# eivindeb/fixed-wing-gym

Hardware: AMD Instinct MI355X
Metric: env-steps/sec (higher is better)
Workload: dtype f32

## Files before the change

fixed-wing-gym_amd/csrc/fwgym.hip:

```cpp
#include <math.h>
#include <stdio.h>
#include <string.h>
#include <string>
#include <vector>
#include "fwgym_env.h"
#include "fwgym_actor.h"
#include "fwgym_learner.h"
#include "fwgym_eval.h"

__device__ __forceinline__ float wave_sum(float v) { return wave_sum64(v); }

struct SpecWords { unsigned w[sizeof(DevCfg) / 4]; };
static_assert(sizeof(SpecWords) == sizeof(DevCfg), "DevCfg must be made of 32-bit members only");
#if defined(FWG_SPECS_FILE)
#include FWG_SPECS_FILE
#elif defined(FWG_WITH_SPECS)
#include "generated/specs.inc"
#else
#define FWG_SPEC_LIST(X)
#endif
#ifndef FWG_SHAPE_LIST
#define FWG_SHAPE_LIST(X)
#endif
#define FWG_SHAPE_BASE FWG_INSTANCE_SHAPE
// ... 1053 lines not shown
    return rollout_shared_floats(c, hsplit) + actor_scratch_floats() + FWG_RO_ENVS * 4;
}
template <bool TURB, int SPEC, int HSPLIT>
__global__ __launch_bounds__(2 * FWG_RO_ENVS, 2) void k_rollout(const DevCfg* __restrict__ cp, const DynCfg* __restrict__ dp, const KArgs A0,
                                                                 const ActorArgs AA) {
    extern __shared__ __attribute__((aligned(16))) float lds[];
    const DevCfg& c = SpecCfg<SPEC>::get(cp);
    constexpr int NK1 = (SpecCfg<SPEC>::obs_dim + 15) / 16;
    const int shared = rollout_shared_floats(c, HSPLIT);
    ActorLds Z;
    Z.F = reinterpret_cast<frag_t*>(lds);
    Z.mean_s = lds + shared;
    Z.rstd_s = Z.mean_s + FWG_ACT_MAX_OBS;
    Z.misc = Z.rstd_s + FWG_ACT_MAX_OBS;
    Z.bias = Z.misc + 4 + 2 * FWG_ACT_MAX_OBS + 4;
    Z.act_out = lds + shared + actor_scratch_floats();
    const unsigned act_ctr = actor_block<HSPLIT, NK1>(AA, Z, (long)blockIdx.x * FWG_RO_ENVS);
    FWG_BLOCK_SYNC_LDS();
    const int wave = threadIdx.x >> 6, group = wave & (FWG_RO_GROUPS - 1);
    const int sub = (int)blockIdx.x * FWG_RO_GROUPS + group;
    const HeadStats hs{Z.mean_s, Z.misc[1], act_ctr + 1u};
    float* area = lds + group * lds_map(c.obs_dim, c.n_obs, c.L.window, c.use_cmd_ring, false, c.obs_log, true).total;
    const float* acts = Z.act_out + group * (FWG_WAVE * 4);
    if (wave < FWG_RO_GROUPS) step_wave<TURB, SPEC, 1, HeadStats>(cp, dp, A0, area, sub, acts, hs);
    else step_wave<TURB, SPEC, 2, HeadStats>(cp, dp, A0, area, sub, acts, hs);
}

template <bool TURB, int SPEC>
__global__ __launch_bounds__(FWG_WAVE) void k_reset(const DevCfg* __restrict__ cp, const DynCfg* __restrict__ dp, const KArgs A0) {
    extern __shared__ __attribute__((aligned(16))) float lds[];
// ... 894 lines not shown
    return FWG_OK;
}

int fwg_reduce_success_device(fwg_handle* h, float* out_dev, void* stream) {
    if (!h || !out_dev) return fail_with(FWG_ERR_INVALID, "null argument");
    launch_finish(h, h->last_metrics_out, (hipStream_t)stream);
    hipLaunchKernelGGL(k_reduce_take, dim3(1), dim3(FWG_WAVE), 0, (hipStream_t)stream, h->d_reduce, out_dev);
    HIP_TRY(hipGetLastError());
    return FWG_OK;
}

int fwg_spec_index(const fwg_handle* h) { return h ? h->spec : -1; }
#ifdef FWG_TIMELINE
int fwg_debug_set_trace(fwg_handle* h, long long* trace_dev) { if (!h) return FWG_ERR_INVALID; h->trace = trace_dev; return FWG_OK; }
int fwg_debug_set_actor_trace(struct fwg_actor* a, long long* trace_dev);
#endif

int fwg_set_graph_mode(fwg_handle* h, int enable, void* stream) {
    if (!h) return fail_with(FWG_ERR_INVALID, "null handle");
    HIP_TRY(hipStreamSynchronize((hipStream_t)stream));
    if (enable) {
        StepSlots s[2];
        s[h->gstep & 1] = host_slots(h, h->gstep);
        s[(h->gstep + 1) & 1] = host_slots(h, h->gstep - 1);
        HIP_TRY(hipMemcpy(h->d_slots, s, sizeof(s), hipMemcpyHostToDevice));
    } else if (h->graph_mode) {
        StepSlots s[2];
        HIP_TRY(hipMemcpy(s, h->d_slots, sizeof(s), hipMemcpyDeviceToHost));
        h->gstep = s[0].gnow > s[1].gnow ? s[0].gnow : s[1].gnow;
    }
// ... 89 lines not shown
static void launch(const fwg_handle* h, const KArgs& A, hipStream_t stream) {
    if (with_instance(h->spec, [&](auto inst) { launch_one<IS_STEP, decltype(inst)::TURB, decltype(inst)::SPEC>(h, A, stream); })) return;
#ifndef FWG_DEV_FAST_BUILD
    if (h->h.turbulence) launch_one<IS_STEP, true, -1>(h, A, stream);
    else launch_one<IS_STEP, false, -1>(h, A, stream);
#endif
}


struct fwg_actor {
    int device;
    int64_t n_envs, env_base;
    int D, act_dim, nk1;
    float gamma, clip_obs, clip_rew, eps;
    int training, precise, parity;
    uint64_t seed;
    ActorStats* d_stats;
    unsigned long long* d_acc;
    int acc_cols;
    frag_t* d_frags;
    float* d_bias;
    float* d_log_std;
    float* d_ret;
    size_t lds_act[2];
    int cnn_filters, cnn_rows;
    size_t lds_cnn[2];
    const fwg_handle* log_env;
#ifdef FWG_TIMELINE
    long long* trace;
#endif
// ... 26 lines not shown

static ActorArgs act_args(const fwg_actor* a, const float* obs, const float* reward, const uint8_t* done, float* norm_obs_out, float* action_out,
                          float* value_out, float* logp_out, float* norm_reward_out, uint8_t* done_out, int deterministic) {
    ActorArgs A = actor_args(a);
    A.obs = obs; A.rew = reward; A.done = done;
    A.norm_obs = norm_obs_out; A.action = action_out; A.value = value_out; A.logp = logp_out; A.norm_rew = norm_reward_out;
    A.done_out = done_out; A.deterministic = deterministic ? 1 : 0;
    return A;
}
typedef void (*actor_kernel_t)(ActorArgs);
static actor_kernel_t actor_kernel(int precise, int nk1) {
    static const actor_kernel_t table[2][4] = {{k_actor_act<1, 1>, k_actor_act<1, 2>, k_actor_act<1, 3>, k_actor_act<1, 4>},
                                               {k_actor_act<3, 1>, k_actor_act<3, 2>, k_actor_act<3, 3>, k_actor_act<3, 4>}};
    return table[precise ? 1 : 0][nk1 - 1];
}

static bool rollout_fits(const fwg_handle* h);
static bool rollout_grant_lds(const fwg_handle* h);

static void observer_args(const fwg_handle* h, KArgs* A) {
    const fwg_actor* a = h->observer;
    if (!a) return;
    A->acc = a->d_acc;
    A->acc_ctr = &a->d_stats[a->parity].act_counter;
    A->acc_mean = a->d_stats[a->parity].mean; A->acc_ret_mean = &a->d_stats[a->parity].ret_mean;
    A->acc_ret = a->d_ret; A->acc_gamma = a->gamma; A->acc_cols = a->acc_cols;
}

extern "C" {

int fwg_attach_observer(fwg_handle* h, fwg_actor* a) {
    if (!h) return fail_with(FWG_ERR_INVALID, "fwg_attach_observer: null env handle");
    if (a && h->h.obs_log > 0)
        return fail_with(FWG_ERR_INVALID, "fwg_attach_observer: row-log observations keep the lagged rows out of the step kernel; use fwg_actor_observe");
    if (a && (a->n_envs != h->n_envs || a->D != h->h.obs_dim || a->device != h->device))
        return fail_with(FWG_ERR_INVALID, "fwg_attach_observer: the head was created for another batch size / observation size / device");
    h->observer = a;
    h->rollout_lds_granted = 0;
    if (a && h->spec >= 0 && h->split && rollout_fits(h)) h->rollout_lds_granted = rollout_grant_lds(h) ? 1 : 0;
    return FWG_OK;
}

#ifdef FWG_TIMELINE
int fwg_debug_set_actor_trace(fwg_actor* a, long long* trace_dev) { if (!a) return FWG_ERR_INVALID; a->trace = trace_dev; return FWG_OK; }
#endif
int fwg_actor_set_obs_log(fwg_actor* a, const fwg_handle* env) {
    if (!a) return fail_with(FWG_ERR_INVALID, "fwg_actor_set_obs_log: null actor");
    if (env != nullptr) {
        if (env->h.obs_log <= 0) return fail_with(FWG_ERR_INVALID, "fwg_actor_set_obs_log: the env writes the dense observation batch");
        if (env->n_envs != a->n_envs || env->h.obs_dim != a->D || env->device != a->device || (env->h.n_obs & 3))
            return fail_with(FWG_ERR_INVALID, "fwg_actor_set_obs_log: batch size / observation size / device mismatch (n_obs must be a multiple of 4)");
        if (a->cnn_filters && env->h.n_obs * a->cnn_rows != a->D)
            return fail_with(FWG_ERR_INVALID, "fwg_actor_set_obs_log: the CNN head's conv spans a window of another length than the env's");
    }
    a->log_env = env;
    return FWG_OK;
}

int fwg_actor_create(int device, int64_t n_envs, int obs_dim, int act_dim, float gamma, float clip_obs, float clip_reward,
                     float epsilon, fwg_actor** out) {
    if (!out) return fail_with(FWG_ERR_INVALID, "fwg_actor_create: null argument");
    if (n_envs < 1) return fail_with(FWG_ERR_INVALID, "fwg_actor_create: n_envs < 1");
    if (obs_dim < 1 || obs_dim > FWG_ACT_MAX_OBS) return fail_with(FWG_ERR_INVALID, "fwg_actor_create: obs_dim must be in [1, 64]");
    if (act_dim < 1 || act_dim > FWG_ACT_MAX_ACT) return fail_with(FWG_ERR_INVALID, "fwg_actor_create: act_dim must be in [1, 4]");
    HIP_TRY(hipSetDevice(device));
    fwg_actor* a = new fwg_actor();
    memset(a, 0, sizeof(*a));
    a->device = device; a->n_envs = n_envs; a->D = obs_dim; a->act_dim = act_dim; a->nk1 = (obs_dim + 15) / 16;
    a->gamma = gamma; a->clip_obs = clip_obs; a->clip_rew = clip_reward; a->eps = epsilon;
    a->training = 1; a->precise = 1;
    a->acc_cols = acc_cols_for(obs_dim);
    a->lds_act[0] = actor_lds_bytes(a->nk1, 1);
    a->lds_act[1] = actor_lds_bytes(a->nk1, 2);
    const int rc = [&]() -> int {
        const size_t nfrag = (size_t)2 * 2 * actor_frags(a->nk1) * 64;
        HIP_TRY(hipMalloc((void**)&a->d_stats, 2 * sizeof(ActorStats)));
        const size_t acc_bytes = (size_t)FWG_ACC_SETS * FWG_ACC_SHARDS * a->acc_cols * sizeof(unsigned long long);
        HIP_TRY(hipMalloc((void**)&a->d_acc, acc_bytes));
        HIP_TRY(hipMemset(a->d_acc, 0, acc_bytes));
        HIP_TRY(hipMalloc((void**)&a->d_frags, nfrag * sizeof(frag_t)));
        HIP_TRY(hipMalloc((void**)&a->d_bias, (2 * FWG_ACT_BIAS_FLOATS + FWG_CNN_PARAMS) * sizeof(float)));
        HIP_TRY(hipMemset(a->d_bias, 0, (2 * FWG_ACT_BIAS_FLOATS + FWG_CNN_PARAMS) * sizeof(float)));
        HIP_TRY(hipMalloc((void**)&a->d_log_std, FWG_ACT_MAX_ACT * sizeof(float)));
        HIP_TRY(hipMalloc((void**)&a->d_ret, (size_t)n_envs * sizeof(float)));
        HIP_TRY(hipMemset(a->d_frags, 0, nfrag * sizeof(frag_t)));
        HIP_TRY(hipMemset(a->d_log_std, 0, FWG_ACT_MAX_ACT * sizeof(float)));
        HIP_TRY(hipMemset(a->d_ret, 0, (size_t)n_envs * sizeof(float)));
        ActorStats s[2];
        memset(s, 0, sizeof(s));
        for (int p = 0; p < 2; ++p) {
            for (int f = 0; f < FWG_ACT_MAX_OBS; ++f) s[p].var[f] = 1.f;
            s[p].count = 1e-4f; s[p].ret_var = 1.f; s[p].ret_count = 1e-4f;
        }
        HIP_TRY(hipMemcpy(a->d_stats, s, sizeof(s), hipMemcpyHostToDevice));
        for (int precise = 0; precise < 2; ++precise)
            HIP_TRY(hipFuncSetAttribute((const void*)actor_kernel(precise, a->nk1), hipFuncAttributeMaxDynamicSharedMemorySize, (int)a->lds_act[precise]));
        return FWG_OK;
    }();
    if (rc != FWG_OK) { fwg_actor_destroy(a); return rc; }
    *out = a;
    return FWG_OK;
}

void fwg_actor_destroy(fwg_actor* a) {
    if (!a) return;
    (void)hipFree(a->d_stats); (void)hipFree(a->d_acc); (void)hipFree(a->d_frags); (void)hipFree(a->d_bias); (void)hipFree(a->d_log_std); (void)hipFree(a->d_ret);
    delete a;
}

int fwg_actor_set_weights(fwg_actor* a, const fwg_actor_weights* w) {
    if (!a || !w) return fail_with(FWG_ERR_INVALID, "fwg_actor_set_weights: null argument");
// ... 108 lines not shown
    HIP_TRY(hipGetLastError());
    return FWG_OK;
}

int fwg_actor_act(fwg_actor* a, const float* obs, const float* reward, const uint8_t* done, float* norm_obs_out,
                  float* action_out, float* value_out, float* logp_out, float* norm_reward_out, uint8_t* done_out,
                  int deterministic, void* stream) {
    if (!a || !obs) return fail_with(FWG_ERR_INVALID, "fwg_actor_act: null argument");
    HIP_TRY(hipSetDevice(a->device));
    const ActorArgs A = act_args(a, obs, reward, done, norm_obs_out, action_out, value_out, logp_out, norm_reward_out, done_out, deterministic);
    const dim3 grid((unsigned)((a->n_envs + FWG_ACT_ENVS - 1) / FWG_ACT_ENVS)), block(64 * FWG_ACT_WAVES);
    hipStream_t st = (hipStream_t)stream;
    if (a->cnn_filters) {
        if (a->precise) hipLaunchKernelGGL((k_actor_act_cnn<3>), grid, block, a->lds_cnn[1], st, A);
        else hipLaunchKernelGGL((k_actor_act_cnn<1>), grid, block, a->lds_cnn[0], st, A);
    } else hipLaunchKernelGGL(actor_kernel(a->precise, a->nk1), grid, block, a->lds_act[a->precise], st, A);
    HIP_TRY(hipGetLastError());
    a->parity ^= 1;
    return FWG_OK;
}

}
static size_t rollout_lds_bytes(const fwg_handle* h, int hsplit) { return (size_t)rollout_lds_floats(h->h, hsplit) * sizeof(float); }
static bool rollout_fits(const fwg_handle* h) {
    bool ok = false;
    with_instance(h->spec, [&](auto inst) { ok = SpecCfg<decltype(inst)::SPEC>::rollout_ok && rollout_lds_bytes(h, 3) <= 160 * 1024; });
    return ok;
}
static bool rollout_grant_lds(const fwg_handle* h) {
    bool ok = false;
    with_instance(h->spec, [&](auto inst) {
// ... 180 lines not shown
```

fixed-wing-gym_amd/csrc/fwgym_actor.h:

```cpp
#pragma once
#include "fwgym_env.h"

#define FWG_STREAM_POLICY 6u
#define FWG_ACT_BLOCK 256
#define FWG_ACT_WAVES 8
#define FWG_ACT_ENVS (32 * FWG_ACT_WAVES)
#define FWG_ACT_PRESCALE 2.885390081777927f
#define FWG_ACT_MAX_OBS 64
#define FWG_ACT_MAX_ACT 4

struct ActorStats { float mean[FWG_ACT_MAX_OBS], var[FWG_ACT_MAX_OBS]; float count, ret_mean, ret_var, ret_count; unsigned act_counter, pad_[3]; };

struct alignas(16) frag_t { unsigned x, y, z, w; };

struct ActorArgs {
    const float* obs; const float* rew; const uint8_t* done;
    const StepSlots* obs_slots; long long obs_win; int obs_n;
#ifdef FWG_TIMELINE
    long long* trace;
#endif
    float* ret;
    ActorStats* stats;
    unsigned long long* acc; int acc_cols;
    const frag_t* frags;
// ... 49 lines not shown
    return __uint_as_float(u);
#else
    float f; memcpy(&f, &u, 4); return f;
#endif
}

__device__ __forceinline__ const float* actor_obs_at(const ActorArgs& A, long long win, long e, int f0) {
    if (A.obs_n == 0) return A.obs + e * A.D + f0;
    const int r = f0 / A.obs_n, j = f0 - r * A.obs_n;
    return A.obs + ((win + r) * A.N + e) * A.obs_n + j;
}
__device__ __forceinline__ long long actor_obs_win(const ActorArgs& A) { return A.obs_slots != nullptr ? A.obs_slots->log_win : A.obs_win; }

#ifdef FWG_TIMELINE
#define FWG_ATL(A, i) do { if ((A).trace != nullptr) { const long long t_ = __builtin_amdgcn_s_memtime(); asm volatile("" ::: "memory"); \
        if ((threadIdx.x & 63) == 0) (A).trace[(blockIdx.x * FWG_ACT_WAVES + (threadIdx.x >> 6)) * 16 + (i)] = t_; } } while (0)
#else
#define FWG_ATL(A, i) do { } while (0)
#endif

typedef float f32x16 __attribute__((ext_vector_type(16)));
#ifdef FWG_EMU
#define fwg_mfma_bf16(a, b, c) emu_mfma_f32_32x32x16_bf16((a), (b), (c))
#define fwg_exp2(x) exp2f(x)
#else
typedef __bf16 fwg_bf16x8 __attribute__((ext_vector_type(8)));
__device__ __forceinline__ f32x16 fwg_mfma_bf16(const frag_t& a, const frag_t& b, f32x16 c) {
    return __builtin_amdgcn_mfma_f32_32x32x16_bf16(__builtin_bit_cast(fwg_bf16x8, a), __builtin_bit_cast(fwg_bf16x8, b), c, 0, 0, 0);
}
#define fwg_exp2(x) __builtin_amdgcn_exp2f(x)
#endif
// ... 53 lines not shown
__device__ __forceinline__ void mma3s(const frag_t& a_hi, const frag_t& a_lo, const frag_t& b_hi, const frag_t& b_lo, f32x16& acc, f32x16& acc_a,
                                      f32x16& acc_b) {
    if (SPLIT > 1) {
        acc_a = fwg_mfma_bf16(a_lo, b_hi, acc_a);
        acc_b = fwg_mfma_bf16(a_hi, b_lo, acc_b);
    }
    acc = fwg_mfma_bf16(a_hi, b_hi, acc);
}
template <int SPLIT, int NF>
__device__ __forceinline__ void load_frags(const frag_t* F, int nfw, int base, int l, frag_t (&hi)[NF], frag_t (&lo)[NF]) {
#pragma unroll
    for (int i = 0; i < NF; ++i) {
        hi[i] = F[(base + i) * 64 + l];
        if (SPLIT > 1) lo[i] = F[(nfw + base + i) * 64 + l];
    }
}
__device__ __forceinline__ f32x16 bias_tile(const float* b, int it, int half) {
    f32x16 a;
#pragma unroll
    for (int q = 0; q < 4; ++q) {
        const float4 v = *reinterpret_cast<const float4*>(b + 32 * it + 8 * q + 4 * half);
        a[4 * q] = v.x; a[4 * q + 1] = v.y; a[4 * q + 2] = v.z; a[4 * q + 3] = v.w;
    }
    return a;
}

__device__ __forceinline__ void hidden_block(const f32x16& a, int kb, frag_t& hi, frag_t& lo) {
    float x[8];
#if defined(FWG_ABL_TANH_ID)
#pragma unroll
// ... 83 lines not shown
    for (int kk = 0; kk < 4; ++kk) {
        mma3s<SPLIT>(w3_hi[kk], w3_lo[kk], bp_hi[kk], bp_lo[kk], o_pi, oa, ob);
        hidden_block(kk < 2 ? v0 : v1, kk & 1, bv_hi[kk], bv_lo[kk]);
        FWG_SCHED_MFMA_VALU(SPLIT > 1 ? 3 : 1, SPLIT > 1 ? 16 : 48);
        FWG_SCHED_FENCE();
    }
    FWG_ATL(A, 12);
    load_frags<SPLIT, 4>(FV, nfw, 2 * NK1 + 8, l, w3_hi, w3_lo);
    o_vf = bias_tile(bV + 128, 0, half);
    f32x16 va = {0.f}, vb = {0.f};
#pragma unroll
    for (int kk = 0; kk < 4; ++kk) mma3s<SPLIT>(w3_hi[kk], w3_lo[kk], bv_hi[kk], bv_lo[kk], o_vf, va, vb);
    if (SPLIT > 1) {
#pragma unroll
        for (int i = 0; i < 4; ++i) { o_pi[i] += oa[i] + ob[i]; o_vf[i] += va[i] + vb[i]; }
    }
}

__global__ __launch_bounds__(FWG_ACT_BLOCK) void k_actor_stats(const ActorArgs A) {
    const int tid = threadIdx.x, lane = tid & 63;
    const long e = (long)blockIdx.x * FWG_ACT_BLOCK + tid;
    const bool valid = e < A.N;
    const long wave = e >> 6;
    if ((wave << 6) >= A.N) return;
    const ActorStats& S = A.stats[A.parity];
    const int D = A.D;
    const bool has_obs = A.obs != nullptr, has_ret = A.rew != nullptr;
    float dr = 0.f;
    if (has_ret && valid) {
        const float r = A.ret[e] * A.gamma + A.rew[e];
// ... 8 lines not shown
        float v[32];
#pragma unroll
        for (int i = 0; i < 32; ++i) v[i] = FWG_ACC_COLUMN(32 * chunk + i, D, valid, FWG_OBS_AT, S.mean, dr, has_obs, has_ret);
        acc_flush(acc, A.acc_cols, (int)(wave & (FWG_ACC_SHARDS - 1)), chunk, lane, wave_totals32(v, lane));
    }
#undef FWG_OBS_AT
}

struct ActorLds {
    frag_t* F;
    float* mean_s;
    float* rstd_s;
    float* misc;
    float* act_out;
    float* bias;
};
__host__ __device__ inline int actor_weight_floats(int nk1, int parts) { return 2 * parts * actor_frags(nk1) * 64 * 4; }
__host__ __device__ inline int actor_scratch_floats() { return 2 * FWG_ACT_MAX_OBS + 4 + 2 * FWG_ACT_MAX_OBS + 4 + 2 * FWG_ACT_BIAS_FLOATS; }

template <int SPLIT, int NK1, bool CNN = false>
__device__ __forceinline__ unsigned actor_block(const ActorArgs& A, const ActorLds& Z, long env_first) {
    const int tid = threadIdx.x, l = tid & 63, wv = tid >> 6, j = l & 31, half = l >> 5;
    constexpr int nf = 2 * NK1 + 12;
    constexpr int PARTS = SPLIT > 1 ? 2 : 1;
    const bool first_block = env_first == 0;
    FWG_ATL(A, 0);
    frag_t* F = Z.F;
    float* mean_s = Z.mean_s;
    float* rstd_s = Z.rstd_s;
    float* misc = Z.misc;
    constexpr int n_pieces = PARTS == 2 ? 2 * 2 * nf : 2 * nf;
    constexpr int per_wave = (n_pieces + FWG_ACT_WAVES - 1) / FWG_ACT_WAVES;
    float4 wreg[per_wave];
#ifndef FWG_ABL_ACT_NO_STAGE
#pragma unroll
    for (int i = 0; i < per_wave; ++i) {
        const int q = wv + i * FWG_ACT_WAVES;
        wreg[i] = make_float4(0.f, 0.f, 0.f, 0.f);
        if (q < n_pieces) {
            const int src = PARTS == 2 ? q : ((q / nf) * 2 * nf + (q % nf));
            wreg[i] = reinterpret_cast<const float4*>(A.frags + src * 64)[l];
        }
    }
#endif
    const long e = env_first + wv * 32 + j;
    const bool valid = e < A.N;
    const bool vec4 = (A.D & 3) == 0 && (A.obs_n & 3) == 0;
    const long long win = actor_obs_win(A);
    constexpr int NRAW = CNN ? FWG_CNN_ROWS * FWG_CNN_COLS / 4 : 1;
    float4 raw_w[NRAW];
    float cnn_p[CNN ? FWG_CNN_PARAMS : 1];
    if constexpr (CNN) {
#pragma unroll
        for (int q = 0; q < NRAW; ++q) raw_w[q] = valid ? *reinterpret_cast<const float4*>(actor_obs_at(A, win, e, 4 * q)) : make_float4(0.f, 0.f, 0.f, 0.f);
#pragma unroll
        for (int i = 0; i < FWG_CNN_PARAMS; ++i) cnn_p[i] = A.bias[2 * FWG_ACT_BIAS_FLOATS + i];
    }
    float raw_x[CNN ? 1 : NK1][8];
#pragma unroll
    for (int kk = 0; kk < (CNN ? 0 : NK1); ++kk) {
// ... 2 lines not shown
            const int f0 = k_input(kk, half, 4 * q);
            float v[4] = {0.f, 0.f, 0.f, 0.f};
            if (valid && f0 < A.D) {
                if (vec4) {
                    const float4 g = *reinterpret_cast<const float4*>(actor_obs_at(A, win, e, f0));
                    v[0] = g.x; v[1] = g.y; v[2] = g.z; v[3] = g.w;
                } else {
#pragma unroll
                    for (int i = 0; i < 4; ++i) if (f0 + i < A.D) v[i] = A.obs[e * A.D + f0 + i];
                }
            }
#pragma unroll
            for (int i = 0; i < 4; ++i) raw_x[kk][4 * q + i] = v[i];
        }
    }
    const unsigned act_ctr = A.stats[A.parity].act_counter;
    const float bias_in = tid < 2 * FWG_ACT_BIAS_FLOATS ? A.bias[tid] : 0.f;
    float ls_in[FWG_ACT_MAX_ACT];
#pragma unroll
    for (int i = 0; i < FWG_ACT_MAX_ACT; ++i) ls_in[i] = i < A.act_dim ? A.log_std[i] : 0.f;
    const float rew_in = (A.rew != nullptr && valid) ? A.rew[e] : 0.f;
    const uint8_t done_in = (A.done != nullptr && valid) ? A.done[e] : (uint8_t)0;
    FWG_ATL(A, 1);
    {
        const ActorStats& S0 = A.stats[A.parity];
        ActorStats& S1 = A.stats[A.parity ^ 1];
        const int D = A.D, cols = 2 * D + 4;
        const size_t set_words = (size_t)FWG_ACC_SHARDS * A.acc_cols;
        const unsigned long long* acc = A.acc + (size_t)(act_ctr % FWG_ACC_SETS) * set_words;
        float* tot = misc + 4;
        if (tid < cols) {
            long long sum = 0;
#pragma unroll
            for (int sh = 0; sh < FWG_ACC_SHARDS; ++sh) sum += (long long)acc[(long)sh * A.acc_cols + tid];
            tot[tid] = (tid == 2 || tid == 3) ? (float)sum : (float)sum * (1.f / FWG_ACC_SCALE);
        }
        if (tid < 2 * FWG_ACT_BIAS_FLOATS) Z.bias[tid] = bias_in;
        FWG_BLOCK_SYNC_LDS();
        const float n_obs = A.training ? tot[2] : 0.f, n_ret = A.training ? tot[3] : 0.f;
        if (tid < FWG_ACT_MAX_OBS) {
            const int f = tid;
            float m = 0.f, rs = 0.f, v = 1.f;
            if (f < D) {
                m = S0.mean[f]; v = S0.var[f];
                if (n_obs > 0.f) {
                    const float cnt = S0.count, tt = cnt + n_obs;
                    const float s1 = tot[4 + 2 * f] / n_obs, s2 = tot[5 + 2 * f] / n_obs;
                    const float bvar = fmaxf(s2 - s1 * s1, 0.f);
                    const float mm = v * cnt + bvar * n_obs + s1 * s1 * (cnt * n_obs / tt);
                    m += s1 * (n_obs / tt);
                    v = mm / tt;
                }
                rs = 1.f / sqrtf(v + A.eps);
            }
            mean_s[f] = m; rstd_s[f] = rs;
            if (first_block) { S1.mean[f] = m; S1.var[f] = v; }
        }
        if (tid == FWG_ACT_MAX_OBS) {
            float rm = S0.ret_mean, rv = S0.ret_var, rc = S0.ret_count;
            if (n_ret > 0.f) {
                const float tt = rc + n_ret;
                const float s1 = tot[0] / n_ret, s2 = tot[1] / n_ret;
                const float bvar = fmaxf(s2 - s1 * s1, 0.f);
                const float mm = rv * rc + bvar * n_ret + s1 * s1 * (rc * n_ret / tt);
                rm += s1 * (n_ret / tt);
                rv = mm / tt;
                rc = tt;
            }
            misc[0] = 1.f / sqrtf(rv + A.eps);
            misc[1] = rm;
            if (first_block) {
                S1.count = S0.count + n_obs; S1.ret_mean = rm; S1.ret_var = rv; S1.ret_count = rc;
                S1.act_counter = act_ctr + 1u;
            }
        }
        if (first_block) {
            unsigned long long* nxt = A.acc + (size_t)((act_ctr + 2u) % FWG_ACC_SETS) * set_words;
            for (int i = tid; i < FWG_ACC_SHARDS * A.acc_cols; i += 64 * FWG_ACT_WAVES) nxt[i] = 0ull;
        }
    }
    FWG_BLOCK_SYNC_LDS();
    FWG_ATL(A, 2);

    frag_t bx_hi[NK1], bx_lo[NK1];
    if constexpr (CNN) {
        static_assert(NK1 == FWG_CNN_NK1, "CNN head: layer 0 takes the 36 conv outputs");
        float xn[FWG_CNN_ROWS * FWG_CNN_COLS];
#pragma unroll
        for (int q = 0; q < NRAW; ++q) {
            const float r4[4] = {raw_w[q].x, raw_w[q].y, raw_w[q].z, raw_w[q].w};
#pragma unroll
            for (int i = 0; i < 4; ++i) xn[4 * q + i] = fminf(fmaxf((r4[i] - mean_s[4 * q + i]) * rstd_s[4 * q + i], -A.clip_obs), A.clip_obs);
            if (A.norm_obs != nullptr && valid && (q < NRAW / 2) == (half == 0))
// ... 20 lines not shown
            split8(x, bx_hi[kk], bx_lo[kk]);
        }
    }
#pragma unroll
    for (int kk = 0; kk < (CNN ? 0 : NK1); ++kk) {
        float x[8];
#pragma unroll
        for (int q = 0; q < 2; ++q) {
            const int f0 = k_input(kk, half, 4 * q);
            float v[4] = {raw_x[kk][4 * q], raw_x[kk][4 * q + 1], raw_x[kk][4 * q + 2], raw_x[kk][4 * q + 3]};
#pragma unroll
            for (int i = 0; i < 4; ++i) {
                v[i] = fminf(fmaxf((v[i] - mean_s[f0 + i]) * rstd_s[f0 + i], -A.clip_obs), A.clip_obs);
                x[4 * q + i] = v[i];
            }
            if (A.norm_obs != nullptr && valid && f0 < A.D) {
                if (vec4) *reinterpret_cast<float4*>(A.norm_obs + e * A.D + f0) = make_float4(v[0], v[1], v[2], v[3]);
                else {
#pragma unroll
                    for (int i = 0; i < 4; ++i) if (f0 + i < A.D) A.norm_obs[e * A.D + f0 + i] = v[i];
                }
            }
        }
        split8(x, bx_hi[kk], bx_lo[kk]);
    }
    FWG_ATL(A, 3);
#ifndef FWG_ABL_ACT_NO_STAGE
#pragma unroll
    for (int i = 0; i < per_wave; ++i) {
        const int q = wv + i * FWG_ACT_WAVES;
        if (q < n_pieces) reinterpret_cast<float4*>(F + q * 64)[l] = wreg[i];
    }
#endif
    float noise_n[4] = {0.f, 0.f, 0.f, 0.f}, noise_s[FWG_ACT_MAX_ACT] = {0.f, 0.f, 0.f, 0.f}, lp = 0.f;
    if (half == 0) {
        if (!A.deterministic) {
            const u4 b = philox4x32((unsigned)(A.env_base + e), act_ctr, 0u, FWG_STREAM_POLICY, A.seed_lo, A.seed_hi);
            box_muller(b, noise_n);
        }
#pragma unroll
        for (int i = 0; i < FWG_ACT_MAX_ACT; ++i) {
            if (i < A.act_dim) {
                const float ls = ls_in[i];
                noise_s[i] = expf(ls) * noise_n[i];
                lp += -0.5f * noise_n[i] * noise_n[i] - ls - 0.9189385332046727f;
            }
        }
    }
    FWG_BLOCK_SYNC_LDS();
    FWG_ATL(A, 4);
#ifdef FWG_ABL_ACT_NO_MLP
    f32x16 o_pi = {0.f}, o_vf = {0.f};
    o_pi[0] = __uint_as_float(bx_hi[0].x ^ F[l].x); o_vf[0] = __uint_as_float(bx_lo[0].y);
#else
    f32x16 o_pi, o_vf;
    mlp_pair<SPLIT, NK1>(A, F, F + PARTS * nf * 64, Z.bias, Z.bias + FWG_ACT_BIAS_FLOATS, l, bx_hi, bx_lo, o_pi, o_vf);
#endif
    FWG_ATL(A, 5);
    const float res[2][FWG_ACT_MAX_ACT] = {{o_pi[0], o_pi[1], o_pi[2], o_pi[3]}, {o_vf[0], o_vf[1], o_vf[2], o_vf[3]}};
    if (half == 0) {
        float act[FWG_ACT_MAX_ACT] = {0.f, 0.f, 0.f, 0.f};
#pragma unroll
        for (int i = 0; i < FWG_ACT_MAX_ACT; ++i) {
            if (i < A.act_dim) {
                act[i] = res[0][i] + noise_s[i];
                if (A.action != nullptr && valid) A.action[e * A.act_dim + i] = act[i];
            }
        }
        if (Z.act_out != nullptr) *reinterpret_cast<float4*>(Z.act_out + (wv * 32 + j) * 4) = make_float4(act[0], act[1], act[2], act[3]);
        if (valid) {
            if (A.logp != nullptr) A.logp[e] = lp;
            if (A.value != nullptr) A.value[e] = res[1][0];
            if (A.norm_rew != nullptr && A.rew != nullptr)
                A.norm_rew[e] = fminf(fmaxf(rew_in * misc[0], -A.clip_rew), A.clip_rew);
            if (A.done_out != nullptr && A.done != nullptr) A.done_out[e] = done_in;
        }
    }
    FWG_ATL(A, 6);
    return act_ctr;
}

template <int SPLIT, int NK1>
__global__ __launch_bounds__(64 * FWG_ACT_WAVES) void k_actor_act(const ActorArgs A) {
    extern __shared__ __attribute__((aligned(16))) float lds[];
    constexpr int PARTS = SPLIT > 1 ? 2 : 1;
    ActorLds Z;
    Z.F = reinterpret_cast<frag_t*>(lds);
    Z.mean_s = lds + actor_weight_floats(NK1, PARTS);
    Z.rstd_s = Z.mean_s + FWG_ACT_MAX_OBS;
    Z.misc = Z.rstd_s + FWG_ACT_MAX_OBS;
    Z.act_out = nullptr;
    Z.bias = Z.misc + 4 + 2 * FWG_ACT_MAX_OBS + 4;
    actor_block<SPLIT, NK1>(A, Z, (long)blockIdx.x * FWG_ACT_ENVS);
}

template <int SPLIT>
__global__ __launch_bounds__(64 * FWG_ACT_WAVES) void k_actor_act_cnn(const ActorArgs A) {
    extern __shared__ __attribute__((aligned(16))) float lds[];
    constexpr int PARTS = SPLIT > 1 ? 2 : 1;
    ActorLds Z;
    Z.F = reinterpret_cast<frag_t*>(lds);
    Z.mean_s = lds + actor_weight_floats(FWG_CNN_NK1, PARTS);
    Z.rstd_s = Z.mean_s + FWG_ACT_MAX_OBS;
    Z.misc = Z.rstd_s + FWG_ACT_MAX_OBS;
    Z.act_out = nullptr;
    Z.bias = Z.misc + 4 + 2 * FWG_ACT_MAX_OBS + 4;
    actor_block<SPLIT, FWG_CNN_NK1, true>(A, Z, (long)blockIdx.x * FWG_ACT_ENVS);
}

static void actor_pack_layer(std::vector<unsigned>& hi, std::vector<unsigned>& lo, const float* W, int out,
                             int in, int nit, int nk, bool chained, float scale) {
    for (int it = 0; it < nit; ++it)
        for (int kk = 0; kk < nk; ++kk)
            for (int l = 0; l < 64; ++l) {
                unsigned wh[4] = {0, 0, 0, 0}, wl[4] = {0, 0, 0, 0};
                const int i = 32 * it + (l & 31), half = l >> 5;
                for (int t = 0; t < 8; ++t) {
                    float v = 0.f;
                    const int k = chained ? k_chained(kk, half, t) : k_input(kk, half, t);
                    if (i < out && k < in) v = scale * W[(size_t)i * in + k];
                    const unsigned h16 = bf16_rne(v), l16 = bf16_rne(v - bf16_to_f32(h16));
// ... 13 lines not shown
```

Baseline: 6.017 billion.

## Split actor head across separate policy and value waves, prefetch stats earlier

Adds a wide actor kernel variant, enabled by default, that launches twice as many waves per block. Each wave evaluates only the policy MLP or only the value MLP for its 32 envs, instead of one wave evaluating both. The loads of the accumulator shards, running stats and weight staging are moved ahead of the first barrier, and noise generation is hoisted earlier to overlap with memory latency. This trades more threads and some duplicated observation loading and normalisation for a shorter per-wave MLP critical path. It also adds an env var to choose 8 or 16 waves.

After: 6.003 billion. No clear change (-0.2%).

```diff
diff --git a/fixed-wing-gym_amd/csrc/fwgym.hip b/fixed-wing-gym_amd/csrc/fwgym.hip
--- a/fixed-wing-gym_amd/csrc/fwgym.hip
+++ b/fixed-wing-gym_amd/csrc/fwgym.hip
@@ -1091,6 +1091,7 @@
     Z.rstd_s = Z.mean_s + FWG_ACT_MAX_OBS;
     Z.misc = Z.rstd_s + FWG_ACT_MAX_OBS;
     Z.bias = Z.misc + 4 + 2 * FWG_ACT_MAX_OBS + 4;
+    Z.s0 = Z.bias + 2 * FWG_ACT_BIAS_FLOATS;
     Z.act_out = lds + shared + actor_scratch_floats();
     const unsigned act_ctr = actor_block<HSPLIT, NK1>(AA, Z, (long)blockIdx.x * FWG_RO_ENVS);
     FWG_BLOCK_SYNC_LDS();
@@ -2015,6 +2016,7 @@
 #ifdef FWG_TIMELINE
 int fwg_debug_set_trace(fwg_handle* h, long long* trace_dev) { if (!h) return FWG_ERR_INVALID; h->trace = trace_dev; return FWG_OK; }
 int fwg_debug_set_actor_trace(struct fwg_actor* a, long long* trace_dev);
+int fwg_debug_actor_waves(const struct fwg_actor* a);
 #endif
 
 int fwg_set_graph_mode(fwg_handle* h, int enable, void* stream) {
@@ -2134,6 +2136,7 @@
     int D, act_dim, nk1;
     float gamma, clip_obs, clip_rew, eps;
     int training, precise, parity;
+    int wide;
     uint64_t seed;
     ActorStats* d_stats;
     unsigned long long* d_acc;
@@ -2190,6 +2193,16 @@
                                                {k_actor_act<3, 1>, k_actor_act<3, 2>, k_actor_act<3, 3>, k_actor_act<3, 4>}};
     return table[precise ? 1 : 0][nk1 - 1];
 }
+static actor_kernel_t actor_kernel_wide(int precise, int nk1) {
+    static const actor_kernel_t table[2][4] = {{k_actor_act<1, 1, 2>, k_actor_act<1, 2, 2>, k_actor_act<1, 3, 2>, k_actor_act<1, 4, 2>},
+                                               {k_actor_act<3, 1, 2>, k_actor_act<3, 2, 2>, k_actor_act<3, 3, 2>, k_actor_act<3, 4, 2>}};
+    return table[precise ? 1 : 0][nk1 - 1];
+}
+static actor_kernel_t actor_kernel_for(const fwg_actor* a, int precise, int* waves) {
+    actor_kernel_t k = a->wide ? actor_kernel_wide(precise, a->nk1) : nullptr;
+    *waves = k ? 2 * FWG_ACT_WAVES : FWG_ACT_WAVES;
+    return k ? k : actor_kernel(precise, a->nk1);
+}
 
 static bool rollout_fits(const fwg_handle* h);
 static bool rollout_grant_lds(const fwg_handle* h);
@@ -2219,6 +2232,11 @@
 
 #ifdef FWG_TIMELINE
 int fwg_debug_set_actor_trace(fwg_actor* a, long long* trace_dev) { if (!a) return FWG_ERR_INVALID; a->trace = trace_dev; return FWG_OK; }
+int fwg_debug_actor_waves(const fwg_actor* a) {
+    int waves = FWG_ACT_WAVES;
+    if (a && !a->cnn_filters) (void)actor_kernel_for(a, a->precise, &waves);
+    return waves;
+}
 #endif
 int fwg_actor_set_obs_log(fwg_actor* a, const fwg_handle* env) {
     if (!a) return fail_with(FWG_ERR_INVALID, "fwg_actor_set_obs_log: null actor");
@@ -2245,6 +2263,14 @@
     a->device = device; a->n_envs = n_envs; a->D = obs_dim; a->act_dim = act_dim; a->nk1 = (obs_dim + 15) / 16;
     a->gamma = gamma; a->clip_obs = clip_obs; a->clip_rew = clip_reward; a->eps = epsilon;
     a->training = 1; a->precise = 1;
+    {
+        const char* env = getenv("FWGYM_HEAD_WAVES");
+        if (env != nullptr && strcmp(env, "8") != 0 && strcmp(env, "16") != 0) {
+            delete a;
+            return fail_with(FWG_ERR_INVALID, "fwg_actor_create: FWGYM_HEAD_WAVES must be 8 or 16");
+        }
+        a->wide = !(env != nullptr && env[0] == '8');
+    }
     a->acc_cols = acc_cols_for(obs_dim);
     a->lds_act[0] = actor_lds_bytes(a->nk1, 1);
     a->lds_act[1] = actor_lds_bytes(a->nk1, 2);
@@ -2269,8 +2295,10 @@
             s[p].count = 1e-4f; s[p].ret_var = 1.f; s[p].ret_count = 1e-4f;
         }
         HIP_TRY(hipMemcpy(a->d_stats, s, sizeof(s), hipMemcpyHostToDevice));
-        for (int precise = 0; precise < 2; ++precise)
-            HIP_TRY(hipFuncSetAttribute((const void*)actor_kernel(precise, a->nk1), hipFuncAttributeMaxDynamicSharedMemorySize, (int)a->lds_act[precise]));
+        for (int precise = 0; precise < 2; ++precise) {
+            int waves;
+            HIP_TRY(hipFuncSetAttribute((const void*)actor_kernel_for(a, precise, &waves), hipFuncAttributeMaxDynamicSharedMemorySize, (int)a->lds_act[precise]));
+        }
         return FWG_OK;
     }();
     if (rc != FWG_OK) { fwg_actor_destroy(a); return rc; }
@@ -2409,7 +2437,11 @@
     if (a->cnn_filters) {
         if (a->precise) hipLaunchKernelGGL((k_actor_act_cnn<3>), grid, block, a->lds_cnn[1], st, A);
         else hipLaunchKernelGGL((k_actor_act_cnn<1>), grid, block, a->lds_cnn[0], st, A);
-    } else hipLaunchKernelGGL(actor_kernel(a->precise, a->nk1), grid, block, a->lds_act[a->precise], st, A);
+    } else {
+        int waves;
+        const actor_kernel_t k = actor_kernel_for(a, a->precise, &waves);
+        hipLaunchKernelGGL(k, grid, dim3(64 * waves), a->lds_act[a->precise], st, A);
+    }
     HIP_TRY(hipGetLastError());
     a->parity ^= 1;
     return FWG_OK;
diff --git a/fixed-wing-gym_amd/csrc/fwgym_actor.h b/fixed-wing-gym_amd/csrc/fwgym_actor.h
--- a/fixed-wing-gym_amd/csrc/fwgym_actor.h
+++ b/fixed-wing-gym_amd/csrc/fwgym_actor.h
@@ -87,7 +87,7 @@
 
 #ifdef FWG_TIMELINE
 #define FWG_ATL(A, i) do { if ((A).trace != nullptr) { const long long t_ = __builtin_amdgcn_s_memtime(); asm volatile("" ::: "memory"); \
-        if ((threadIdx.x & 63) == 0) (A).trace[(blockIdx.x * FWG_ACT_WAVES + (threadIdx.x >> 6)) * 16 + (i)] = t_; } } while (0)
+        if ((threadIdx.x & 63) == 0) (A).trace[(blockIdx.x * (blockDim.x >> 6) + (threadIdx.x >> 6)) * 16 + (i)] = t_; } } while (0)
 #else
 #define FWG_ATL(A, i) do { } while (0)
 #endif
@@ -171,6 +171,11 @@
         hi[i] = F[(base + i) * 64 + l];
         if (SPLIT > 1) lo[i] = F[(nfw + base + i) * 64 + l];
     }
+}
+template <int SPLIT>
+__device__ __forceinline__ void load_frag(const frag_t* F, int nfw, int i, int l, frag_t& hi, frag_t& lo) {
+    hi = F[i * 64 + l];
+    if (SPLIT > 1) lo = F[(nfw + i) * 64 + l];
 }
 __device__ __forceinline__ f32x16 bias_tile(const float* b, int it, int half) {
     f32x16 a;
@@ -284,6 +289,56 @@
     if (SPLIT > 1) {
 #pragma unroll
         for (int i = 0; i < 4; ++i) { o_pi[i] += oa[i] + ob[i]; o_vf[i] += va[i] + vb[i]; }
+    }
+}
+
+template <int SPLIT, int NK1>
+__device__ __forceinline__ void mlp_one(const frag_t* F, const float* b, int l, const frag_t (&bx_hi)[NK1], const frag_t (&bx_lo)[NK1], f32x16& out) {
+    constexpr int nfw = 2 * NK1 + 12;
+    const int half = l >> 5;
+    frag_t wa_hi[2], wa_lo[2], wb_hi[2], wb_lo[2];
+    f32x16 p0 = bias_tile(b, 0, half), p1 = bias_tile(b, 1, half);
+    load_frag<SPLIT>(F, nfw, 0, l, wa_hi[0], wa_lo[0]);
+    load_frag<SPLIT>(F, nfw, NK1, l, wb_hi[0], wb_lo[0]);
+#pragma unroll
+    for (int kk = 0; kk < NK1; ++kk) {
+        const int c = kk & 1, n = c ^ 1;
+        if (kk + 1 < NK1) {
+            load_frag<SPLIT>(F, nfw, kk + 1, l, wa_hi[n], wa_lo[n]);
+            load_frag<SPLIT>(F, nfw, NK1 + kk + 1, l, wb_hi[n], wb_lo[n]);
+        } else {
+            load_frag<SPLIT>(F, nfw, 2 * NK1, l, wa_hi[n], wa_lo[n]);
+            load_frag<SPLIT>(F, nfw, 2 * NK1 + 4, l, wb_hi[n], wb_lo[n]);
+        }
+        mma3x2<SPLIT>(wa_hi[c], wa_lo[c], wb_hi[c], wb_lo[c], bx_hi[kk], bx_lo[kk], p0, p1);
+    }
+    constexpr int c0 = NK1 & 1;
+    f32x16 h0 = bias_tile(b + 64, 0, half), h1 = bias_tile(b + 64, 1, half);
+    frag_t bh_hi[4], bh_lo[4];
+    hidden_block(p0, 0, bh_hi[0], bh_lo[0]);
+#pragma unroll
+    for (int kk = 0; kk < 4; ++kk) {
+        const int c = (c0 + kk) & 1, n = c ^ 1;
+        if (kk + 1 < 4) {
+            load_frag<SPLIT>(F, nfw, 2 * NK1 + kk + 1, l, wa_hi[n], wa_lo[n]);
+            load_frag<SPLIT>(F, nfw, 2 * NK1 + 4 + kk + 1, l, wb_hi[n], wb_lo[n]);
+            hidden_block(kk + 1 < 2 ? p0 : p1, (kk + 1) & 1, bh_hi[kk + 1], bh_lo[kk + 1]);
+        }
+        mma3x2<SPLIT>(wa_hi[c], wa_lo[c], wb_hi[c], wb_lo[c], bh_hi[kk], bh_lo[kk], h0, h1);
+    }
+    frag_t w3_hi[4], w3_lo[4];
+    load_frags<SPLIT, 4>(F, nfw, 2 * NK1 + 8, l, w3_hi, w3_lo);
+    out = bias_tile(b + 128, 0, half);
+    f32x16 oa = {0.f}, ob = {0.f};
+    hidden_block(h0, 0, bh_hi[0], bh_lo[0]);
+#pragma unroll
+    for (int kk = 0; kk < 4; ++kk) {
+        if (kk + 1 < 4) hidden_block(kk + 1 < 2 ? h0 : h1, (kk + 1) & 1, bh_hi[kk + 1], bh_lo[kk + 1]);
+        mma3s<SPLIT>(w3_hi[kk], w3_lo[kk], bh_hi[kk], bh_lo[kk], out, oa, ob);
+    }
+    if (SPLIT > 1) {
+#pragma unroll
+        for (int i = 0; i < 4; ++i) out[i] += oa[i] + ob[i];
     }
 }
 
@@ -322,13 +377,18 @@
     float* misc;
     float* act_out;
     float* bias;
+    float* s0;
 };
 __host__ __device__ inline int actor_weight_floats(int nk1, int parts) { return 2 * parts * actor_frags(nk1) * 64 * 4; }
-__host__ __device__ inline int actor_scratch_floats() { return 2 * FWG_ACT_MAX_OBS + 4 + 2 * FWG_ACT_MAX_OBS + 4 + 2 * FWG_ACT_BIAS_FLOATS; }
-
-template <int SPLIT, int NK1, bool CNN = false>
+__host__ __device__ inline int actor_scratch_floats() { return 2 * FWG_ACT_MAX_OBS + 4 + 2 * FWG_ACT_MAX_OBS + 4 + 2 * FWG_ACT_BIAS_FLOATS + 4; }
+
+template <int SPLIT, int NK1, bool CNN = false, int WPT = 1>
 __device__ __forceinline__ unsigned actor_block(const ActorArgs& A, const ActorLds& Z, long env_first) {
+    static_assert(WPT == 1 || (WPT == 2 && !CNN), "a wave per network: the MLP head's own launch only");
+    constexpr int NW = FWG_ACT_WAVES * WPT;
     const int tid = threadIdx.x, l = tid & 63, wv = tid >> 6, j = l & 31, half = l >> 5;
+    const int tile = WPT == 1 ? wv : (wv & (FWG_ACT_WAVES - 1));
+    const bool is_pi = WPT == 1 || wv < FWG_ACT_WAVES, is_vf = WPT == 1 || wv >= FWG_ACT_WAVES;
     constexpr int nf = 2 * NK1 + 12;
     constexpr int PARTS = SPLIT > 1 ? 2 : 1;
     const bool first_block = env_first == 0;
@@ -337,21 +397,7 @@
     float* mean_s = Z.mean_s;
     float* rstd_s = Z.rstd_s;
     float* misc = Z.misc;
-    constexpr int n_pieces = PARTS == 2 ? 2 * 2 * nf : 2 * nf;
-    constexpr int per_wave = (n_pieces + FWG_ACT_WAVES - 1) / FWG_ACT_WAVES;
-    float4 wreg[per_wave];
-#ifndef FWG_ABL_ACT_NO_STAGE
-#pragma unroll
-    for (int i = 0; i < per_wave; ++i) {
-        const int q = wv + i * FWG_ACT_WAVES;
-        wreg[i] = make_float4(0.f, 0.f, 0.f, 0.f);
-        if (q < n_pieces) {
-            const int src = PARTS == 2 ? q : ((q / nf) * 2 * nf + (q % nf));
-            wreg[i] = reinterpret_cast<const float4*>(A.frags + src * 64)[l];
-        }
-    }
-#endif
-    const long e = env_first + wv * 32 + j;
+    const long e = env_first + tile * 32 + j;
     const bool valid = e < A.N;
     const bool vec4 = (A.D & 3) == 0 && (A.obs_n & 3) == 0;
     const long long win = actor_obs_win(A);
@@ -384,37 +430,81 @@
             for (int i = 0; i < 4; ++i) raw_x[kk][4 * q + i] = v[i];
         }
     }
-    const unsigned act_ctr = A.stats[A.parity].act_counter;
+    const ActorStats& S0 = A.stats[A.parity];
+    const unsigned act_ctr = S0.act_counter;
+    static_assert(FWG_ACC_SETS == 3 && FWG_ACC_SETS * (2 * FWG_ACT_MAX_OBS + 4) <= 64 * NW, "one lane per (set, column)");
+    const int cols = 2 * A.D + 4;
+    const int acc_set = (tid >= cols ? 1 : 0) + (tid >= 2 * cols ? 1 : 0), acc_col = tid - acc_set * cols;
+    const size_t set_words = (size_t)FWG_ACC_SHARDS * A.acc_cols;
+    unsigned long long shard_in[FWG_ACC_SHARDS];
+#pragma unroll
+    for (int sh = 0; sh < FWG_ACC_SHARDS; ++sh) shard_in[sh] = 0ull;
+    if (tid < FWG_ACC_SETS * cols) {
+        const unsigned long long* acc = A.acc + (size_t)acc_set * set_words + acc_col;
+#pragma unroll
+        for (int sh = 0; sh < FWG_ACC_SHARDS; ++sh) shard_in[sh] = acc[(long)sh * A.acc_cols];
+    }
+    float s0_mean = 0.f, s0_var = 1.f, s0_aux = 0.f;
+    if (tid < FWG_ACT_MAX_OBS) { s0_mean = S0.mean[tid]; s0_var = S0.var[tid]; }
+    else if (tid < FWG_ACT_MAX_OBS + 4) s0_aux = (&S0.count)[tid - FWG_ACT_MAX_OBS];
+    constexpr int n_pieces = PARTS == 2 ? 2 * 2 * nf : 2 * nf;
+    constexpr int per_wave = (n_pieces + NW - 1) / NW;
+    float4 wreg[per_wave];
+#ifndef FWG_ABL_ACT_NO_STAGE
+#pragma unroll
+    for (int i = 0; i < per_wave; ++i) {
+        const int q = wv + i * NW;
+        wreg[i] = make_float4(0.f, 0.f, 0.f, 0.f);
+        if (q < n_pieces) {
+            const int src = PARTS == 2 ? q : ((q / nf) * 2 * nf + (q % nf));
+            wreg[i] = reinterpret_cast<const float4*>(A.frags + src * 64)[l];
+        }
+    }
+#endif
     const float bias_in = tid < 2 * FWG_ACT_BIAS_FLOATS ? A.bias[tid] : 0.f;
     float ls_in[FWG_ACT_MAX_ACT];
 #pragma unroll
     for (int i = 0; i < FWG_ACT_MAX_ACT; ++i) ls_in[i] = i < A.act_dim ? A.log_std[i] : 0.f;
-    const float rew_in = (A.rew != nullptr && valid) ? A.rew[e] : 0.f;
-    const uint8_t done_in = (A.done != nullptr && valid) ? A.done[e] : (uint8_t)0;
+    const float rew_in = (is_vf && A.rew != nullptr && valid) ? A.rew[e] : 0.f;
+    const uint8_t done_in = (is_vf && A.done != nullptr && valid) ? A.done[e] : (uint8_t)0;
     FWG_ATL(A, 1);
+    float noise_n[4] = {0.f, 0.f, 0.f, 0.f}, noise_s[FWG_ACT_MAX_ACT] = {0.f, 0.f, 0.f, 0.f}, lp = 0.f;
+    if (is_pi && half == 0) {
+        if (!A.deterministic) {
+            const u4 b = philox4x32((unsigned)(A.env_base + e), act_ctr, 0u, FWG_STREAM_POLICY, A.seed_lo, A.seed_hi);
+            box_muller(b, noise_n);
+        }
+#pragma unroll
+        for (int i = 0; i < FWG_ACT_MAX_ACT; ++i) {
+            if (i < A.act_dim) {
+                const float ls = ls_in[i];
+                noise_s[i] = expf(ls) * noise_n[i];
+                lp += -0.5f * noise_n[i] * noise_n[i] - ls - 0.9189385332046727f;
+            }
+        }
+    }
     {
-        const ActorStats& S0 = A.stats[A.parity];
         ActorStats& S1 = A.stats[A.parity ^ 1];
-        const int D = A.D, cols = 2 * D + 4;
-        const size_t set_words = (size_t)FWG_ACC_SHARDS * A.acc_cols;
-        const unsigned long long* acc = A.acc + (size_t)(act_ctr % FWG_ACC_SETS) * set_words;
+        const int D = A.D;
         float* tot = misc + 4;
-        if (tid < cols) {
+        if (tid < FWG_ACC_SETS * cols && acc_set == (int)(act_ctr % FWG_ACC_SETS)) {
             long long sum = 0;
 #pragma unroll
-            for (int sh = 0; sh < FWG_ACC_SHARDS; ++sh) sum += (long long)acc[(long)sh * A.acc_cols + tid];
-            tot[tid] = (tid == 2 || tid == 3) ? (float)sum : (float)sum * (1.f / FWG_ACC_SCALE);
+            for (int sh = 0; sh < FWG_ACC_SHARDS; ++sh) sum += (long long)shard_in[sh];
+            tot[acc_col] = (acc_col == 2 || acc_col == 3) ? (float)sum : (float)sum * (1.f / FWG_ACC_SCALE);
         }
         if (tid < 2 * FWG_ACT_BIAS_FLOATS) Z.bias[tid] = bias_in;
+        if (tid >= FWG_ACT_MAX_OBS && tid < FWG_ACT_MAX_OBS + 4) Z.s0[tid - FWG_ACT_MAX_OBS] = s0_aux;
         FWG_BLOCK_SYNC_LDS();
         const float n_obs = A.training ? tot[2] : 0.f, n_ret = A.training ? tot[3] : 0.f;
+        const float s0_count = Z.s0[0];
         if (tid < FWG_ACT_MAX_OBS) {
             const int f = tid;
             float m = 0.f, rs = 0.f, v = 1.f;
             if (f < D) {
-                m = S0.mean[f]; v = S0.var[f];
+                m = s0_mean; v = s0_var;
                 if (n_obs > 0.f) {
-                    const float cnt = S0.count, tt = cnt + n_obs;
+                    const float cnt = s0_count, tt = cnt + n_obs;
                     const float s1 = tot[4 + 2 * f] / n_obs, s2 = tot[5 + 2 * f] / n_obs;
                     const float bvar = fmaxf(s2 - s1 * s1, 0.f);
                     const float mm = v * cnt + bvar * n_obs + s1 * s1 * (cnt * n_obs / tt);
@@ -427,7 +517,7 @@
             if (first_block) { S1.mean[f] = m; S1.var[f] = v; }
         }
         if (tid == FWG_ACT_MAX_OBS) {
-            float rm = S0.ret_mean, rv = S0.ret_var, rc = S0.ret_count;
+            float rm = Z.s0[1], rv = Z.s0[2], rc = Z.s0[3];
             if (n_ret > 0.f) {
                 const float tt = rc + n_ret;
                 const float s1 = tot[0] / n_ret, s2 = tot[1] / n_ret;
@@ -440,13 +530,13 @@
             misc[0] = 1.f / sqrtf(rv + A.eps);
             misc[1] = rm;
             if (first_block) {
-                S1.count = S0.count + n_obs; S1.ret_mean = rm; S1.ret_var = rv; S1.ret_count = rc;
+                S1.count = s0_count + n_obs; S1.ret_mean = rm; S1.ret_var = rv; S1.ret_count = rc;
                 S1.act_counter = act_ctr + 1u;
             }
         }
         if (first_block) {
             unsigned long long* nxt = A.acc + (size_t)((act_ctr + 2u) % FWG_ACC_SETS) * set_words;
-            for (int i = tid; i < FWG_ACC_SHARDS * A.acc_cols; i += 64 * FWG_ACT_WAVES) nxt[i] = 0ull;
+            for (int i = tid; i < FWG_ACC_SHARDS * A.acc_cols; i += 64 * NW) nxt[i] = 0ull;
         }
     }
     FWG_BLOCK_SYNC_LDS();
@@ -497,7 +587,7 @@
                 v[i] = fminf(fmaxf((v[i] - mean_s[f0 + i]) * rstd_s[f0 + i], -A.clip_obs), A.clip_obs);
                 x[4 * q + i] = v[i];
             }
-            if (A.norm_obs != nullptr && valid && f0 < A.D) {
+            if (is_pi && A.norm_obs != nullptr && valid && f0 < A.D) {
                 if (vec4) *reinterpret_cast<float4*>(A.norm_obs + e * A.D + f0) = make_float4(v[0], v[1], v[2], v[3]);
                 else {
 #pragma unroll
@@ -511,25 +601,10 @@
 #ifndef FWG_ABL_ACT_NO_STAGE
 #pragma unroll
     for (int i = 0; i < per_wave; ++i) {
-        const int q = wv + i * FWG_ACT_WAVES;
+        const int q = wv + i * NW;
         if (q < n_pieces) reinterpret_cast<float4*>(F + q * 64)[l] = wreg[i];
     }
 #endif
-    float noise_n[4] = {0.f, 0.f, 0.f, 0.f}, noise_s[FWG_ACT_MAX_ACT] = {0.f, 0.f, 0.f, 0.f}, lp = 0.f;
-    if (half == 0) {
-        if (!A.deterministic) {
-            const u4 b = philox4x32((unsigned)(A.env_base + e), act_ctr, 0u, FWG_STREAM_POLICY, A.seed_lo, A.seed_hi);
-            box_muller(b, noise_n);
-        }
-#pragma unroll
-        for (int i = 0; i < FWG_ACT_MAX_ACT; ++i) {
-            if (i < A.act_dim) {
-                const float ls = ls_in[i];
-                noise_s[i] = expf(ls) * noise_n[i];
-                lp += -0.5f * noise_n[i] * noise_n[i] - ls - 0.9189385332046727f;
-            }
-        }
-    }
     FWG_BLOCK_SYNC_LDS();
     FWG_ATL(A, 4);
 #ifdef FWG_ABL_ACT_NO_MLP
@@ -537,11 +612,15 @@
     o_pi[0] = __uint_as_float(bx_hi[0].x ^ F[l].x); o_vf[0] = __uint_as_float(bx_lo[0].y);
 #else
     f32x16 o_pi, o_vf;
-    mlp_pair<SPLIT, NK1>(A, F, F + PARTS * nf * 64, Z.bias, Z.bias + FWG_ACT_BIAS_FLOATS, l, bx_hi, bx_lo, o_pi, o_vf);
+    if constexpr (WPT == 1) mlp_pair<SPLIT, NK1>(A, F, F + PARTS * nf * 64, Z.bias, Z.bias + FWG_ACT_BIAS_FLOATS, l, bx_hi, bx_lo, o_pi, o_vf);
+    else {
+        mlp_one<SPLIT, NK1>(F + (is_vf ? PARTS * nf * 64 : 0), Z.bias + (is_vf ? FWG_ACT_BIAS_FLOATS : 0), l, bx_hi, bx_lo, o_pi);
+        o_vf = o_pi;
+    }
 #endif
     FWG_ATL(A, 5);
     const float res[2][FWG_ACT_MAX_ACT] = {{o_pi[0], o_pi[1], o_pi[2], o_pi[3]}, {o_vf[0], o_vf[1], o_vf[2], o_vf[3]}};
-    if (half == 0) {
+    if (is_pi && half == 0) {
         float act[FWG_ACT_MAX_ACT] = {0.f, 0.f, 0.f, 0.f};
 #pragma unroll
         for (int i = 0; i < FWG_ACT_MAX_ACT; ++i) {
@@ -550,9 +629,11 @@
                 if (A.action != nullptr && valid) A.action[e * A.act_dim + i] = act[i];
             }
         }
-        if (Z.act_out != nullptr) *reinterpret_cast<float4*>(Z.act_out + (wv * 32 + j) * 4) = make_float4(act[0], act[1], act[2], act[3]);
+        if (Z.act_out != nullptr) *reinterpret_cast<float4*>(Z.act_out + (tile * 32 + j) * 4) = make_float4(act[0], act[1], act[2], act[3]);
+        if (A.logp != nullptr && valid) A.logp[e] = lp;
+    }
+    if (is_vf && half == 0) {
         if (valid) {
-            if (A.logp != nullptr) A.logp[e] = lp;
             if (A.value != nullptr) A.value[e] = res[1][0];
             if (A.norm_rew != nullptr && A.rew != nullptr)
                 A.norm_rew[e] = fminf(fmaxf(rew_in * misc[0], -A.clip_rew), A.clip_rew);
@@ -563,8 +644,8 @@
     return act_ctr;
 }
 
-template <int SPLIT, int NK1>
-__global__ __launch_bounds__(64 * FWG_ACT_WAVES) void k_actor_act(const ActorArgs A) {
+template <int SPLIT, int NK1, int WPT = 1>
+__global__ __launch_bounds__(64 * FWG_ACT_WAVES * WPT) void k_actor_act(const ActorArgs A) {
     extern __shared__ __attribute__((aligned(16))) float lds[];
     constexpr int PARTS = SPLIT > 1 ? 2 : 1;
     ActorLds Z;
@@ -574,7 +655,8 @@
     Z.misc = Z.rstd_s + FWG_ACT_MAX_OBS;
     Z.act_out = nullptr;
     Z.bias = Z.misc + 4 + 2 * FWG_ACT_MAX_OBS + 4;
-    actor_block<SPLIT, NK1>(A, Z, (long)blockIdx.x * FWG_ACT_ENVS);
+    Z.s0 = Z.bias + 2 * FWG_ACT_BIAS_FLOATS;
+    actor_block<SPLIT, NK1, false, WPT>(A, Z, (long)blockIdx.x * FWG_ACT_ENVS);
 }
 
 template <int SPLIT>
@@ -588,6 +670,7 @@
     Z.misc = Z.rstd_s + FWG_ACT_MAX_OBS;
     Z.act_out = nullptr;
     Z.bias = Z.misc + 4 + 2 * FWG_ACT_MAX_OBS + 4;
+    Z.s0 = Z.bias + 2 * FWG_ACT_BIAS_FLOATS;
     actor_block<SPLIT, FWG_CNN_NK1, true>(A, Z, (long)blockIdx.x * FWG_ACT_ENVS);
 }
 
```
